# omahs/cess

Measured on AMD Instinct MI355X. Metric: verified BLS12-381 sigs/sec (node), higher is better.
Workload: dtype u32 (381-bit Montgomery, 14x28-bit limb products via v_mad_u64_u32)

## Files before the change

cess_amd/csrc/bls/pair.hpp:

```cpp
#pragma once
#include "staged.hpp"
#include "../kernels.hpp"

#if !defined(CESS_HOSTEMU)
namespace bls {

CESS_HD uint32_t dpp_swap(uint32_t x) { return (uint32_t)__builtin_amdgcn_mov_dpp((int)x, 0xB1, 0xF, 0xF, true); }
CESS_HD uint32_t dpp_even(uint32_t x) { return (uint32_t)__builtin_amdgcn_mov_dpp((int)x, 0xA0, 0xF, 0xF, true); }
CESS_HD uint32_t dpp_odd(uint32_t x) { return (uint32_t)__builtin_amdgcn_mov_dpp((int)x, 0xF5, 0xF, 0xF, true); }

CESS_HD uint32_t pair_hi_mask() { return 0u - (__lane_id() & 1u); }

struct fph {
  fp v;
};
struct fp6h {
  fph c0, c1, c2;
};

CESS_HD fph fph_of(const fp& v) { return {v}; }
CESS_HD fph add(const fph& a, const fph& b) { return {add(a.v, b.v)}; }
CESS_HD fph sub(const fph& a, const fph& b) { return {sub(a.v, b.v)}; }
CESS_HD fph add_nr(const fph& a, const fph& b) { return {add_nr(a.v, b.v)}; }
CESS_HD fph dbl(const fph& a) { return {dbl(a.v)}; }
CESS_HD fph neg(const fph& a) { return {neg(a.v)}; }
CESS_HD fp xchg(const fp& a) {
  fp r;
#pragma unroll
  for (int i = 0; i < 12; i++) r.v[i] = dpp_swap(a.v[i]);
  return r;
}
CESS_HD fp partner_signed(const fp& own) {
  const fp p = xchg(own);
  const uint32_t hm = pair_hi_mask();
  fp r;
  uint32_t bw = 0;
#pragma unroll
  for (int i = 0; i < 12; i++) {
    const uint32_t n = subc32(c::P2_RAW[i], p.v[i], bw, &bw);
    r.v[i] = (p.v[i] & hm) | (n & ~hm);
  }
  return r;
}
CESS_HD fph mul_nr(const fph& a) { return {add(a.v, partner_signed(a.v))}; }
CESS_HD fph mul_nr_nr(const fph& a) { return {add_nr(a.v, partner_signed(a.v))}; }
CESS_HD fph add_xi_nr(const fph& a, const fph& b) { return {add_nr(add_nr(a.v, b.v), partner_signed(b.v))}; }
CESS_HD bool pair_and(bool b) {
  const uint32_t x = b ? 1u : 0u;
  return (x & dpp_swap(x)) != 0;
}
CESS_HD bool is_zero(const fph& a) { return pair_and(is_zero(a.v)); }
CESS_HD bool eq(const fph& a, const fph& b) { return pair_and(eq(a.v, b.v)); }
CESS_HD fph select(bool c, const fph& a, const fph& b) { return {select(c, a.v, b.v)}; }
CESS_HD fph mul3(const fph& a) { return {mul3(a.v)}; }
CESS_HD fph fph_one() {
  const uint32_t hm = pair_hi_mask();
  fp r;
#pragma unroll
  for (int i = 0; i < 12; i++) r.v[i] = c::ONE[i] & ~hm;
  return {r};
}
CESS_HD fph fph_zero() { return {fp_zero()}; }
CESS_HD fph conj(const fph& a) {
  const fp n = neg(a.v);
  const uint32_t hm = pair_hi_mask();
  fp r;
#pragma unroll
  for (int i = 0; i < 12; i++) r.v[i] = (n.v[i] & hm) | (a.v.v[i] & ~hm);
  return {r};
}

template <uint32_t S = 1>
CESS_HD void pair_digits(const fp& a, const fp& b, uint32_t (&xa)[14], uint32_t (&xb)[14], uint32_t (&ya)[14],
                         uint32_t (&yb)[14]) {
  uint32_t yo[14];
  unpack28(a, xa);
  unpack28(b, yo);
  const uint32_t hm = pair_hi_mask();
#pragma unroll
  for (int i = 0; i < 14; i++) {
    if (S != 1) xa[i] *= S;
    xb[i] = dpp_swap(xa[i]);
    ya[i] = dpp_even(yo[i]);
    const uint32_t t = dpp_odd(yo[i]);
    yb[i] = (t & hm) | ((c::NEG_K28[i] - t) & ~hm);
  }
}

template <uint32_t S>
CESS_HD fph pmul_scaled(const fph& a0, const fph& b0) {
  static_assert(S >= 1 && S <= 3, "digit bound");
  CESS_COUNT_MUL2();
  fp a = a0.v, b = b0.v;
  seq(a);
  seq(b);
  uint32_t xa[14], xb[14], ya[14], yb[14];
  pair_digits<S>(a, b, xa, xb, ya, yb);
  fp r = mont28([&](int k, uint64_t& acc) {
#pragma unroll
    for (int i = 0; i < 14; i++) {
      const int j = k - i;
      if (j < 0 || j >= 14) continue;
      mac(acc, xa[i], ya[j]);
      mac(acc, xb[i], yb[j]);
    }
  });
  seq(r);
  return {r};
}
CESS_HD fph pmul(const fph& a, const fph& b) { return pmul_scaled<1>(a, b); }

CESS_HD fph psqr(const fph& a) {
  const fp p = xchg(a.v);
  const bool hi = pair_hi_mask() != 0;
  fp x, y;
  uint32_t cx = 0, bn = 0, cy = 0;
#pragma unroll
  for (int i = 0; i < 12; i++) {
    x.v[i] = addc32(a.v.v[i], hi ? a.v.v[i] : p.v[i], cx, &cx);
    const uint32_t n = subc32(c::P2_RAW[i], p.v[i], bn, &bn);
    const uint32_t t = addc32(a.v.v[i], n, cy, &cy);
    y.v[i] = hi ? p.v[i] : t;
  }
  return {mul(x, y)};
}

CESS_HD fph pinv(const fph& a) {
  const fp n = sqr(a.v);
  const fp t = inv(add(n, xchg(n)));
  return conj(fph{mul(a.v, t)});
}

CESS_HD fph pdot2(const fph& a0, const fph& b0, const fph& c0, const fph& d0) {
  CESS_COUNT_HALVES(8);
  fp a = a0.v, b = b0.v, c = c0.v, d = d0.v;
  seq(a);
  seq(b);
  seq(c);
  seq(d);
  uint32_t xa[14], xb[14], ya[14], yb[14], ua[14], ub[14], wa[14], wb[14];
  pair_digits(a, b, xa, xb, ya, yb);
  pair_digits(c, d, ua, ub, wa, wb);
  fp r = mont28([&](int k, uint64_t& acc) {
#pragma unroll
    for (int i = 0; i < 14; i++) {
      const int j = k - i;
      if (j < 0 || j >= 14) continue;
      mac(acc, xa[i], ya[j]);
      mac(acc, xb[i], yb[j]);
      mac(acc, ua[i], wa[j]);
      mac(acc, ub[i], wb[j]);
    }
  });
  seq(r);
  return {r};
}

struct pxd {
  uint32_t a[14], b[14];
};
struct pyd {
  uint32_t a[14], b[14];
};
CESS_HD pxd prep_x(const fph& x0) {
  fp x = x0.v;
  seq(x);
  pxd r;
  unpack28(x, r.a);
#pragma unroll
  for (int i = 0; i < 14; i++) r.b[i] = dpp_swap(r.a[i]);
  return r;
}
CESS_HD pyd prep_y(const fph& y0) {
  fp y = y0.v;
  seq(y);
  uint32_t yo[14];
  unpack28(y, yo);
  const uint32_t hm = pair_hi_mask();
  pyd r;
#pragma unroll
  for (int i = 0; i < 14; i++) {
    r.a[i] = dpp_even(yo[i]);
    const uint32_t t = dpp_odd(yo[i]);
    r.b[i] = (t & hm) | ((c::NEG_K28[i] - t) & ~hm);
  }
  return r;
}
CESS_HD fph pmul_p(const pxd& x, const pyd& y) {
  CESS_COUNT_MUL2();
  fp r = mont28([&](int k, uint64_t& acc) {
#pragma unroll
    for (int i = 0; i < 14; i++) {
      const int j = k - i;
      if (j < 0 || j >= 14) continue;
      mac(acc, x.a[i], y.a[j]);
      mac(acc, x.b[i], y.b[j]);
    }
  });
  seq(r);
  return {r};
}
CESS_HD fph pdot2_p(const pxd& x, const pyd& y, const pxd& u, const pyd& w) {
  CESS_COUNT_HALVES(8);
  fp r = mont28([&](int k, uint64_t& acc) {
#pragma unroll
    for (int i = 0; i < 14; i++) {
      const int j = k - i;
      if (j < 0 || j >= 14) continue;
      mac(acc, x.a[i], y.a[j]);
      mac(acc, x.b[i], y.b[j]);
      mac(acc, u.a[i], w.a[j]);
      mac(acc, u.b[i], w.b[j]);
    }
  });
  seq(r);
  return {r};
}

CESS_HD fph pmul_fp(const fph& a, const fp& s) { return {mul(a.v, s)}; }

CESS_HD fp6h add(const fp6h& a, const fp6h& b) { return {add(a.c0, b.c0), add(a.c1, b.c1), add(a.c2, b.c2)}; }
CESS_HD fp6h sub(const fp6h& a, const fp6h& b) { return {sub(a.c0, b.c0), sub(a.c1, b.c1), sub(a.c2, b.c2)}; }
CESS_HD fp6h dbl(const fp6h& a) { return {dbl(a.c0), dbl(a.c1), dbl(a.c2)}; }
CESS_HD fp6h add_nr(const fp6h& a, const fp6h& b) {
  return {add_nr(a.c0, b.c0), add_nr(a.c1, b.c1), add_nr(a.c2, b.c2)};
}
CESS_HD fp6h mul_v(const fp6h& a) { return {mul_nr(a.c2), a.c0, a.c1}; }

CESS_HD fp6h pmul6(const fp6h& a, const fp6h& b) {
  const fph t0 = pmul(a.c0, b.c0);
  const fph t1 = pmul(a.c1, b.c1);
  const fph t2 = pmul(a.c2, b.c2);
  const fph c0 = add(mul_nr(sub(sub(pmul(add_nr(a.c1, a.c2), add_nr(b.c1, b.c2)), t1), t2)), t0);
  const fph c1 = add(sub(sub(pmul(add_nr(a.c0, a.c1), add_nr(b.c0, b.c1)), t0), t1), mul_nr(t2));
  const fph c2 = add(sub(sub(pmul(add_nr(a.c0, a.c2), add_nr(b.c0, b.c2)), t0), t2), t1);
  return {c0, c1, c2};
}
CESS_HD fp6h pmul_by_1(const fp6h& a, const fph& b1) {
  const pyd y = prep_y(b1);
  const fph p2 = pmul_p(prep_x(a.c2), y);
  CESS_MEMBAR();
  const fph p0 = pmul_p(prep_x(a.c0), y);
  CESS_MEMBAR();
  return {mul_nr(p2), p0, pmul_p(prep_x(a.c1), y)};
}

struct LdsPair {
  uint4 (*G)[CESS_PAIR_THREADS];
  uint32_t w0;
  CESS_HD fph ld(int k) const {
    const uint32_t t = w0 + lane_fresh();
    fph r;
#pragma unroll
    for (int q = 0; q < 3; q++) {
      const uint4 x = G[3 * k + q][t];
      r.v.v[4 * q] = x.x, r.v.v[4 * q + 1] = x.y, r.v.v[4 * q + 2] = x.z, r.v.v[4 * q + 3] = x.w;
    }
    return r;
  }
  CESS_HD void st(int k, const fph& a) const {
    const uint32_t t = w0 + lane_fresh();
#pragma unroll
    for (int q = 0; q < 3; q++) G[3 * k + q][t] = make_uint4(a.v.v[4 * q], a.v.v[4 * q + 1], a.v.v[4 * q + 2], a.v.v[4 * q + 3]);
  }
};

template <class S>
CESS_HD fp6h pld6(const S& s, int h) {
  return {s.ld(3 * h), s.ld(3 * h + 1), s.ld(3 * h + 2)};
}
template <class S>
CESS_HD void pst6(const S& s, int h, const fp6h& a) {
  s.st(3 * h, a.c0);
  s.st(3 * h + 1, a.c1);
  s.st(3 * h + 2, a.c2);
}

template <class S>
CESS_HD void psqr12(const S& f) {
  fp6h ab;
#pragma unroll 1
  for (int it = 0; it < 2; it++) {
    const fp6h a0 = pld6(f, 0), a1 = pld6(f, 1);
    fp6h A = a0, B = a1;
    if (it) {
      A = add_nr(a0, a1);
      B = add_nr(a0, mul_v(a1));
    }
    const fp6h r = pmul6(A, B);
    CESS_MEMBAR();
    if (it == 0) {
      ab = r;
    } else {
      pst6(f, 0, sub(sub(r, ab), mul_v(ab)));
      pst6(f, 1, dbl(ab));
    }
  }
}

template <class S>
CESS_HD fp6h pmul_by_01_dot(const S& f, int h, const fph& b0, const fph& b1, const fph& xb1) {
  const pyd y0 = prep_y(b0);
  fp6h r;
  {
    const pxd x0 = prep_x(f.ld(3 * h));
    r.c0 = pdot2_p(x0, y0, prep_x(f.ld(3 * h + 2)), prep_y(xb1));
    CESS_MEMBAR();
    r.c1 = pdot2_p(x0, prep_y(b1), prep_x(f.ld(3 * h + 1)), y0);
  }
  CESS_MEMBAR();
  r.c2 = pdot2_p(prep_x(f.ld(3 * h + 1)), prep_y(b1), prep_x(f.ld(3 * h + 2)), y0);
  return r;
}

template <class S>
CESS_HD void pmul014(const S& f, const fph& c0, const fph& c1, const fph& c4) {
  const fp6h bb = pmul_by_1(pld6(f, 1), c4);
  CESS_MEMBAR();
  const fp6h aa = pmul_by_01_dot(f, 0, c0, c1, mul_nr_nr(c1));
  CESS_MEMBAR();
  pst6(f, 1, add(pld6(f, 0), pld6(f, 1)));
  pst6(f, 0, add(mul_v(bb), aa));
  const fp6h u = add(aa, bb);
  CESS_MEMBAR();
  const fph d = add(c1, c4);
  const fp6h t = pmul_by_01_dot(f, 1, c0, d, mul_nr_nr(d));
  pst6(f, 1, sub(t, u));
}

CESS_HD fp6h pmul_by_01_one(const fp6h& a, const fph& b1) {
  const pyd y = prep_y(b1);
  const fph p2 = pmul_p(prep_x(a.c2), y);
  CESS_MEMBAR();
  const fph p0 = pmul_p(prep_x(a.c0), y);
  CESS_MEMBAR();
  return {add(a.c0, mul_nr(p2)), add(a.c1, p0), add(a.c2, pmul_p(prep_x(a.c1), y))};
}

template <class S>
CESS_HD void pmul014_one(const S& f, const fph& c1, const fph& c4) {
  const fp6h bb = pmul_by_1(pld6(f, 1), c4);
  CESS_MEMBAR();
  fp6h u;
  const fph d = add(c1, c4);
#pragma unroll 1
  for (int it = 0; it < 2; it++) {
    const fp6h r = pmul_by_01_one(pld6(f, it), it ? d : c1);
    CESS_MEMBAR();
    if (it == 0) {
      pst6(f, 1, add(pld6(f, 0), pld6(f, 1)));
      pst6(f, 0, add(mul_v(bb), r));
      u = add(r, bb);
    } else {
      pst6(f, 1, sub(r, u));
    }
  }
}

template <class S, class Pt, class Src>
CESS_HD void miller_loop2_pair(const S& f, bool use0, bool use1, Pt&& pt, Src&& src, bool norm1) {
  f.st(0, fph_one());
#pragma unroll 1
  for (int k = 1; k < 6; k++) f.st(k, fph_zero());
#pragma unroll 1
  for (int s = 0; s < N_COEFFS; s++) {
#pragma unroll 1
    for (int pair = 0; pair < 2; pair++) {
      const int pr = 1 - pair;
      if (!(pr ? use1 : use0)) continue;
      const g1a p = pt(pr);
      const fph c1 = pmul_fp(src(pr, s, 1), p.x), c4 = pmul_fp(src(pr, s, 0), p.y);
      if (pr && !norm1)
        pmul014(f, src(pr, s, 2), c1, c4);
      else
        pmul014_one(f, c1, c4);
      CESS_MEMBAR();
    }
    if (square_after_step(s)) psqr12(f);
    CESS_MEMBAR();
  }
#pragma unroll 1
  for (int k = 3; k < 6; k++) f.st(k, neg(f.ld(k)));
}

template <int NP, class S, class Pt, class Src>
CESS_HD void miller_loopn_pair(const S& f, uint32_t use, Pt&& pt, Src&& src) {
  f.st(0, fph_one());
#pragma unroll 1
  for (int k = 1; k < 6; k++) f.st(k, fph_zero());
#pragma unroll 1
  for (int s = 0; s < N_COEFFS; s++) {
#pragma unroll 1
    for (int j = 0; j < NP; j++) {
      if (!((use >> j) & 1u)) continue;
      const g1a p = pt(j);
      const fph c1 = pmul_fp(src(j, s, 1), p.x), c4 = pmul_fp(src(j, s, 0), p.y);
      pmul014(f, src(j, s, 2), c1, c4);
      CESS_MEMBAR();
    }
    if (square_after_step(s)) psqr12(f);
    CESS_MEMBAR();
  }
#pragma unroll 1
  for (int k = 3; k < 6; k++) f.st(k, neg(f.ld(k)));
}

}
#endif
```

Before: 3.187 million.

## Replace Fp12 squaring with three Fp6 squarings using fused dot-product kernels

Rewrites psqr12 to compute the Fp12 square as three Fp6 squarings (of a0+a1, a0, a1) instead of two Karatsuba Fp6 multiplications. Each Fp6 square is built from fused Montgomery dot products (psqr_dot, pdot2_p) with precomputed doubled and sign-adjusted operands, so cross terms share a single reduction. The goal is fewer Montgomery reductions and multiplies in the Miller loop's squaring step. In exchange there are extra LDS loads and stores across three iterations and new carry-handling code in prep_s.

Result: no change. 3.192 million, median of 6 (+0.2%).

```diff
diff --git a/cess_amd/csrc/bls/pair.hpp b/cess_amd/csrc/bls/pair.hpp
--- a/cess_amd/csrc/bls/pair.hpp
+++ b/cess_amd/csrc/bls/pair.hpp
@@ -217,6 +217,55 @@
   return {r};
 }
 
+CESS_HD pxd prep_x2(const fph& x0) {
+  fp x = x0.v;
+  seq(x);
+  pxd r;
+  unpack28(x, r.a);
+#pragma unroll
+  for (int i = 0; i < 14; i++) {
+    r.a[i] <<= 1;
+    r.b[i] = dpp_swap(r.a[i]);
+  }
+  return r;
+}
+struct psd {
+  uint32_t x[14], y[14];
+};
+CESS_HD psd prep_s(const fph& a) {
+  const fp p = xchg(a.v);
+  const bool hi = pair_hi_mask() != 0;
+  fp x, y;
+  uint32_t cx = 0, bn = 0, cy = 0;
+#pragma unroll
+  for (int i = 0; i < 12; i++) {
+    x.v[i] = addc32(a.v.v[i], hi ? a.v.v[i] : p.v[i], cx, &cx);
+    const uint32_t n = subc32(c::P2_RAW[i], p.v[i], bn, &bn);
+    const uint32_t t = addc32(a.v.v[i], n, cy, &cy);
+    y.v[i] = hi ? p.v[i] : t;
+  }
+  seq(x);
+  seq(y);
+  psd r;
+  unpack28(x, r.x);
+  unpack28(y, r.y);
+  return r;
+}
+CESS_HD fph psqr_dot(const psd& s, const pxd& x, const pyd& y) {
+  fp r = mont28([&](int k, uint64_t& acc) {
+#pragma unroll
+    for (int i = 0; i < 14; i++) {
+      const int j = k - i;
+      if (j < 0 || j >= 14) continue;
+      mac(acc, s.x[i], s.y[j]);
+      mac(acc, x.a[i], y.a[j]);
+      mac(acc, x.b[i], y.b[j]);
+    }
+  });
+  seq(r);
+  return {r};
+}
+
 CESS_HD fph pmul_fp(const fph& a, const fp& s) { return {mul(a.v, s)}; }
 
 CESS_HD fp6h add(const fp6h& a, const fp6h& b) { return {add(a.c0, b.c0), add(a.c1, b.c1), add(a.c2, b.c2)}; }
@@ -227,15 +276,6 @@
 }
 CESS_HD fp6h mul_v(const fp6h& a) { return {mul_nr(a.c2), a.c0, a.c1}; }
 
-CESS_HD fp6h pmul6(const fp6h& a, const fp6h& b) {
-  const fph t0 = pmul(a.c0, b.c0);
-  const fph t1 = pmul(a.c1, b.c1);
-  const fph t2 = pmul(a.c2, b.c2);
-  const fph c0 = add(mul_nr(sub(sub(pmul(add_nr(a.c1, a.c2), add_nr(b.c1, b.c2)), t1), t2)), t0);
-  const fph c1 = add(sub(sub(pmul(add_nr(a.c0, a.c1), add_nr(b.c0, b.c1)), t0), t1), mul_nr(t2));
-  const fph c2 = add(sub(sub(pmul(add_nr(a.c0, a.c2), add_nr(b.c0, b.c2)), t0), t2), t1);
-  return {c0, c1, c2};
-}
 CESS_HD fp6h pmul_by_1(const fp6h& a, const fph& b1) {
   const pyd y = prep_y(b1);
   const fph p2 = pmul_p(prep_x(a.c2), y);
@@ -243,6 +283,18 @@
   const fph p0 = pmul_p(prep_x(a.c0), y);
   CESS_MEMBAR();
   return {mul_nr(p2), p0, pmul_p(prep_x(a.c1), y)};
+}
+
+CESS_HD fp6h psqr6_dot(const fp6h& a) {
+  const pyd y2 = prep_y(a.c2);
+  fph r0, r1, r2;
+  r0 = psqr_dot(prep_s(a.c0), prep_x2(mul_nr_nr(a.c1)), y2);
+  CESS_MEMBAR();
+  const pxd x0 = prep_x2(a.c0);
+  r2 = psqr_dot(prep_s(a.c1), x0, y2);
+  CESS_MEMBAR();
+  r1 = pdot2_p(x0, prep_y(a.c1), prep_x(mul_nr_nr(a.c2)), y2);
+  return {r0, r1, r2};
 }
 
 struct LdsPair {
@@ -278,22 +330,21 @@
 
 template <class S>
 CESS_HD void psqr12(const S& f) {
-  fp6h ab;
-#pragma unroll 1
-  for (int it = 0; it < 2; it++) {
-    const fp6h a0 = pld6(f, 0), a1 = pld6(f, 1);
-    fp6h A = a0, B = a1;
-    if (it) {
-      A = add_nr(a0, a1);
-      B = add_nr(a0, mul_v(a1));
-    }
-    const fp6h r = pmul6(A, B);
+  fp6h x;
+#pragma unroll 1
+  for (int it = 0; it < 3; it++) {
+    fp6h a = pld6(f, it >> 1);
+    if (it == 0) a = add(a, pld6(f, 1));
+    const fp6h r = psqr6_dot(a);
     CESS_MEMBAR();
     if (it == 0) {
-      ab = r;
+      x = r;
+    } else if (it == 1) {
+      x = sub(x, r);
+      pst6(f, 0, r);
     } else {
-      pst6(f, 0, sub(sub(r, ab), mul_v(ab)));
-      pst6(f, 1, dbl(ab));
+      pst6(f, 1, sub(x, r));
+      pst6(f, 0, add(pld6(f, 0), mul_v(r)));
     }
   }
 }
```
